# fabianschenk/REVO

Hardware: AMD Instinct MI355X
Metric: tracked frames/sec at 640x480, 4-level pyramid; ATE vs reference (higher is better)
Workload: dtype f32

## Files before the change

revo_amd/csrc/revo_host.hip:

```cpp
#include "revo_host_impl.h"

static thread_local std::string g_err;
extern "C" const char* revo_last_error(void) { return g_err.c_str(); }
extern "C" const char* revo_version(void) { return "0.1.0 gfx950"; }
extern "C" void revo_set_error_(const char* msg) { g_err = msg ? msg : ""; }

extern "C" void revo_pyr_settings_default(revo_pyr_settings* s) {
  memset(s, 0, sizeof(*s));
  s->width = 640; s->height = 480;
  s->fx = 517.306408f; s->fy = 516.469215f; s->cx = 318.643040f; s->cy = 255.313989f;
  s->pyr_min_lvl = 2; s->pyr_max_lvl = 0;
  s->canny_threshold1 = 150; s->canny_threshold2 = 100;
  s->depth_min = 0.1f; s->depth_max = 5.2f;
  s->use_edge_hist = 1; s->n_percentage = 0.3f;
  s->hist_patch[0] = 20; s->hist_patch[1] = 10; s->hist_patch[2] = 5;
}
extern "C" void revo_opt_settings_default(revo_opt_settings* s) {
  memset(s, 0, sizeof(*s));
  s->lambda_success_fac = 0.5f; s->lambda_fail_fac = 2.0f;
  const float ed[6] = {30, 20, 10, 5, 5, 5};
  for (int i = 0; i < REVO_L; ++i) {
    s->lambda_initial[i] = 0.f; s->step_size_min[i] = 1e-16f; s->convergence_eps[i] = 0.999f;
    s->max_its_per_lvl[i] = 100; s->edge_distance_lvl[i] = ed[i];
  }
  s->huber_edge = 0.3f;
  s->use_edge_filter = 1;
}
extern "C" void revo_tracker_settings_default(revo_tracker_settings* s) {
  s->check_tracking_results = 1; s->check_init_values = 1; s->n_frames_hist_voting = 3;
  s->histogram_level = 2;
}

static int build_geom(const revo_pyr_settings& s, PyrGeom* g, std::string* why) {
  memset(g, 0, sizeof(*g));
  g->fstride = 1;
  const int L = s.pyr_min_lvl - s.pyr_max_lvl + 1;
  if (s.pyr_max_lvl != 0) { *why = "pyr_max_lvl must be 0 (the reference indexes per-level vectors by level)"; return -1; }
  if (L < 1 || L > REVO_L) { *why = "1..6 pyramid levels supported"; return -1; }
  if (s.width <= 0 || s.height <= 0 || s.width > REVO_MAX_WIDTH || s.height > 2048 ||
      ((s.width + 31) / 32) * ((s.height + 31) / 32) > 2048) {
    *why = "image size must be within 2048 x 2048 and 2048 tiles of 32 x 32 pixels (1920 x 1080 fits, 2048 x 1536 does not)"; return -1;
  }
  if (s.width % (4 << (L - 1)) || s.height % (1 << (L - 1))) {
    *why = "width must be a multiple of 4*2^(levels-1) and height of 2^(levels-1)"; return -1;
  }
  g->n_levels = L;
  { const char* e = getenv("REVO_HYST_BANDED"); g->hyst_force = (e && *e) ? (*e != '0' ? 1 : 0) : -1; }
  g->hyst_heavy_runs = env_int("REVO_HYST_HEAVY_RUNS", 0, 0, 1 << 30);
  g->depth_min = s.depth_min; g->depth_max = s.depth_max;
  double lo = s.canny_threshold1, hi = s.canny_threshold2;
  if (lo > hi) std::swap(lo, hi);
  lo = std::min(32767.0, lo); hi = std::min(32767.0, hi);
  if (lo > 0) lo *= lo;
  if (hi > 0) hi *= hi;
  g->canny_low = (int)std::floor(lo); g->canny_high = (int)std::floor(hi);
  g->use_edge_hist = s.use_edge_hist; g->n_percentage = s.n_percentage;
  int tile = 0, pix = 0, row = 0, col = 0, cc = 0, tiles32 = 0, bands = 0;
  bool bands_fit = true;
  for (int l = 0; l < L; ++l) {
    LevelGeom& v = g->lv[l];
    const float scale = 1.0f / (float)std::pow(2, l);
    if (l == 0) { v.fx = s.fx; v.fy = s.fy; v.cx = s.cx; v.cy = s.cy; v.w = s.width; v.h = s.height; }
    else {
      v.fx = s.fx * scale; v.fy = s.fy * scale; v.cx = s.cx * scale; v.cy = s.cy * scale;
      v.w = (int)((float)s.width * scale); v.h = (int)((float)s.height * scale);
    }
    v.npix = v.w * v.h;
    if (v.npix % 16) { *why = "every level must have a multiple of 16 pixels"; return -1; }
    v.patch = s.hist_patch[l] > 0 ? s.hist_patch[l] : 0;
    if (v.patch > 0) {
      v.hist_w = v.w / v.patch; v.hist_h = v.h / v.patch;
      if (v.hist_w < 1 || v.hist_h < 1 || v.hist_w > 128) { *why = "hist_patch out of range for this level size"; return -1; }
    }
    g->fill_thr[l] = (double)(v.patch * v.patch) * 0.05;
    v.chunk_rows = 32; v.nchunk = (v.h + 31) / 32;
    v.wpr = (v.w + 31) / 32;
    v.nms_block_base = tile; tile += (8 * v.wpr * ((v.h + NMS_ROWS - 1) / NMS_ROWS) + 255) / 256;
    v.pix_base = pix; pix += v.npix;
    v.edt_rows = std::max(1, EDT_ROW_PX / v.w);
    v.edt_block_base = row; row += (v.h + v.edt_rows - 1) / v.edt_rows;
    v.strip_base = col; col += (v.w + 63) / 64;
    v.cc_base = cc; cc += v.w * v.nchunk;
    tiles32 += v.wpr * v.nchunk;
    {
      int unit = v.patch > 0 ? v.patch : 4;
      while (unit % 4) unit *= 2;
      int rows = (env_int("REVO_HYST_BAND_WORDS", 2400, 64, 1 << 20) / v.wpr) / unit * unit;
      if (rows < unit) rows = unit;
      if (rows >= v.h) rows = v.h;
      if ((v.h + rows - 1) / rows > 32) rows = ((v.h + 31) / 32 + unit - 1) / unit * unit;
      v.band_rows = rows;
      v.nbands = (v.h + rows - 1) / rows;
      v.band_base = bands; bands += v.nbands;
      if (v.nbands > 1) g->any_banded = 1;
      const size_t nwb = (size_t)rows * v.wpr;
      if (nwb + (nwb + 2) / 2 + (size_t)(rows + 2) * v.wpr + 2 + 256 > 16384) bands_fit = false;
    }
  }
  g->total_tiles = tiles32;
  g->total_bands = bands_fit ? bands : 0;
  for (int l = 1; l < L; ++l)
    g->lv[l].has_orig = (s.use_edge_hist && g->lv[l].patch > 0 && g->lv[l - 1].patch > 0) ? 1 : 0;
  g->total_nms_blocks = tile; g->total_pix = pix; g->total_edt_blocks = row; g->total_strips = col; g->total_cc = cc;
  return 0;
}

static void build_track_params(const revo_ctx* c, TrackParams* t) {
  memset(t, 0, sizeof(*t));
  t->pyr_min_lvl = c->ps.pyr_min_lvl; t->pyr_max_lvl = c->ps.pyr_max_lvl;
  t->lvl_begin = c->ps.pyr_min_lvl; t->lvl_end = c->ps.pyr_max_lvl;
  t->check_init = c->ts.check_init_values;
  t->lambda_success_fac = c->os.lambda_success_fac; t->lambda_fail_fac = c->os.lambda_fail_fac;
  for (int i = 0; i < REVO_L; ++i) {
    t->lambda_initial[i] = c->os.lambda_initial[i]; t->step_size_min[i] = c->os.step_size_min[i];
    t->convergence_eps[i] = c->os.convergence_eps[i]; t->max_its[i] = c->os.max_its_per_lvl[i];
    t->edge_distance[i] = c->os.edge_distance_lvl[i];
  }
  t->huber_edge = c->os.huber_edge; t->use_edge_filter = c->os.use_edge_filter;
  {
    const char* e = getenv("REVO_TRACK_KSPEC");
    const size_t n = e ? strlen(e) : 0;
    for (int i = 0; i < REVO_L; ++i) {
      int k = i < 2 ? 2 : TRACK_KMAX;
      if (n == 1) k = e[0] - '0'; else if (n > 1) k = e[std::min<size_t>(i, n - 1)] - '0';
      t->kspec[i] = std::max(1, std::min(TRACK_KMAX, k));
    }
  }
  t->redundant_n = env_int("REVO_TRACK_REDUNDANT_BATCH", 400, 0, 1 << 30);
  for (int l = 0; l < c->geom.n_levels; ++l) {
    const LevelGeom& v = c->geom.lv[l];
    t->cam[l].fx = v.fx; t->cam[l].fy = v.fy; t->cam[l].cx = v.cx; t->cam[l].cy = v.cy; t->cam[l].w = v.w; t->cam[l].h = v.h;
  }
}

static int env_track_depth() {
  const char* e = getenv("REVO_TRACK_SERIAL");
  if (e && *e && *e != '0') return 1;
  return env_int("REVO_TRACK_DEPTH", 2, 1, 4);
}
int pick_cluster(const revo_ctx* c, int n_pairs) {
  const int resident = c->num_cus * c->blocks_per_cu;
  const int depth = c->knobs.track_depth;
  const int share = n_pairs == 1 || depth == 1 ? (int)(0.75 * resident) : resident / depth;
  int cl = share / std::max(1, n_pairs);
  if (n_pairs == 1) cl = std::min(cl, 16);
  if (cl > TRACK_MAX_CLUSTER) cl = TRACK_MAX_CLUSTER;
  {
    const int want = n_pairs == 1 ? c->knobs.cluster_one : env_int("REVO_TRACK_CLUSTER", 0, 0, TRACK_MAX_CLUSTER);
    const int hard = std::min(TRACK_MAX_CLUSTER, resident / std::max(1, n_pairs));
    if (want >= 1) cl = std::min(want, std::max(1, hard));
  }
  if (cl < 1) cl = 1;
  return cl;
}

#define TRACK_MAX_DEPTH 4
struct TrackChain {
  std::mutex mu;
  hipEvent_t ev[TRACK_MAX_DEPTH] = {};
  hipStream_t st[TRACK_MAX_DEPTH] = {};
  bool has[TRACK_MAX_DEPTH] = {};
  unsigned long long n = 0;
// ... 332 lines not shown
```

revo_amd/csrc/revo_pyramid.hip:

```cpp
#include "revo_dev.h"
#include "revo_nms_px.h"
#include <type_traits>

namespace {

#ifdef REVO_BUILD_PRIO
#define BUILD_PRIO() __builtin_amdgcn_s_setprio(REVO_BUILD_PRIO)
#else
#define BUILD_PRIO()
#endif

__device__ __forceinline__ int level_of(const PyrGeom& g, int v, int LevelGeom::*base) {
  int l = 0;
#pragma unroll
  for (int k = 1; k < REVO_L; ++k)
    if (k < g.n_levels && v >= g.lv[k].*base) l = k;
  return l;
}
__device__ __forceinline__ int clampi(int v, int lo, int hi) { return v < lo ? lo : (v > hi ? hi : v); }
__device__ __forceinline__ int reflect101(int i, int n) {
  if (i < 0) i = -i;
  if (i >= n) i = 2 * n - 2 - i;
  return i;
}

__device__ __forceinline__ uint32_t gray4(uint32_t a, uint32_t b, uint32_t c) {
  const int B0 = a & 255, G0 = (a >> 8) & 255, R0 = (a >> 16) & 255, B1 = a >> 24;
  const int G1 = b & 255, R1 = (b >> 8) & 255, B2 = (b >> 16) & 255, G2 = b >> 24;
  const int R2 = c & 255, B3 = (c >> 8) & 255, G3 = (c >> 16) & 255, R3 = c >> 24;
  const uint32_t y0 = (uint32_t)(B0 * 1868 + G0 * 9617 + R0 * 4899 + 8192) >> 14;
  const uint32_t y1 = (uint32_t)(B1 * 1868 + G1 * 9617 + R1 * 4899 + 8192) >> 14;
  const uint32_t y2 = (uint32_t)(B2 * 1868 + G2 * 9617 + R2 * 4899 + 8192) >> 14;
  const uint32_t y3 = (uint32_t)(B3 * 1868 + G3 * 9617 + R3 * 4899 + 8192) >> 14;
  return y0 | (y1 << 8) | (y2 << 16) | (y3 << 24);
}
__global__ void __launch_bounds__(256) k_gray_depth(const uint8_t* __restrict__ bgr, const float* __restrict__ depth_f32,
                                                    const uint16_t* __restrict__ depth_u16, float alpha,
                                                    uint8_t* __restrict__ gray, float* __restrict__ depth_out, int npix, int frame0) {
  BUILD_PRIO();
  const int f = frame0 + blockIdx.z;
  const int g16 = blockIdx.x * 256 + threadIdx.x;
  if (g16 * 16 >= npix) return;
  const uint4* src = reinterpret_cast<const uint4*>(bgr + (size_t)f * npix * 3) + (size_t)g16 * 3;
  const uint4 p = src[0], q = src[1], r = src[2];
  reinterpret_cast<uint4*>(gray + (size_t)f * npix)[g16] =
      make_uint4(gray4(p.x, p.y, p.z), gray4(p.w, q.x, q.y), gray4(q.z, q.w, r.x), gray4(r.y, r.z, r.w));
  if (depth_out == depth_f32) return;
  float4* dst = reinterpret_cast<float4*>(depth_out + (size_t)f * npix) + (size_t)g16 * 4;
  if (depth_u16) {
    const uint4* raw = reinterpret_cast<const uint4*>(depth_u16 + (size_t)f * npix) + (size_t)g16 * 2;
    const uint4 u = raw[0], v = raw[1];
    const uint32_t wds[8] = {u.x, u.y, u.z, u.w, v.x, v.y, v.z, v.w};
#pragma unroll
    for (int k = 0; k < 4; ++k) {
      float4 d;
      d.x = (float)(wds[2 * k] & 0xffff) * alpha + 0.0f;
      d.y = (float)(wds[2 * k] >> 16) * alpha + 0.0f;
      d.z = (float)(wds[2 * k + 1] & 0xffff) * alpha + 0.0f;
      d.w = (float)(wds[2 * k + 1] >> 16) * alpha + 0.0f;
      dst[k] = d;
    }
  } else {
    const float4* in = reinterpret_cast<const float4*>(depth_f32 + (size_t)f * npix) + (size_t)g16 * 4;
    const float4 d0 = in[0], d1 = in[1], d2 = in[2], d3 = in[3];
    dst[0] = d0; dst[1] = d1; dst[2] = d2; dst[3] = d3;
  }
}

struct EdgeStage {
  const uint2* cs;
  const unsigned short* epre;
  const int* base;
  float* out;
  int wpr, tiles_total;
};
template <bool GRAY, bool DEPTH, bool STAGE = false>
__global__ void __launch_bounds__(256) k_pyrdown(const uint8_t* __restrict__ src, int sw, int sh, uint8_t* __restrict__ dst,
                                                 int dw, int dh, const float* __restrict__ dsrc, float* __restrict__ ddst, int frame0,
                                                 int fstride, uint8_t* __restrict__ vsrc, float dmin, float dmax, EdgeStage es) {
  BUILD_PRIO();
  static_assert(!STAGE || DEPTH, "staging rides on the depth half");
  const int f = frame0 + fstride * blockIdx.z;
  src += (size_t)f * sw * sh;
  dst += (size_t)f * dw * dh;
// ... 1525 lines not shown
  for (int o = 1; o < 64; o <<= 1) {
    const int v = __shfl_up(incl, o);
    if (lane >= o) incl += v;
  }
  if (lane == 63) s_part[wave] = incl;
  __syncthreads();
  int run = incl - sum, total = 0;
#pragma unroll
  for (int k = 0; k < 16; ++k) {
    const int wv = s_part[k];
    run += k < wave ? wv : 0;
    total += wv;
  }
  for (int i = b; i < e; ++i) { const int c = a[i]; a[i] = run; run += c; }
  return total;
}


__global__ void __launch_bounds__(256) k_pyrdown_bgr(const uint8_t* __restrict__ src, int w, int h,
                                                     uint8_t* __restrict__ dst) {
  const int dw = w >> 1, dh = h >> 1;
  const int i = blockIdx.x * 256 + threadIdx.x;
  if (i >= dw * dh) return;
  const int x = i % dw, y = i / dw;
  const int kk[5] = {1, 4, 6, 4, 1};
  int acc[3] = {0, 0, 0};
#pragma unroll
  for (int j = 0; j < 5; ++j) {
    const uint8_t* row = src + (size_t)reflect101(2 * y + j - 2, h) * w * 3;
    int rs[3] = {0, 0, 0};
#pragma unroll
    for (int t = 0; t < 5; ++t) {
      const uint8_t* px = row + (size_t)reflect101(2 * x + t - 2, w) * 3;
      rs[0] += kk[t] * px[0]; rs[1] += kk[t] * px[1]; rs[2] += kk[t] * px[2];
    }
    acc[0] += kk[j] * rs[0]; acc[1] += kk[j] * rs[1]; acc[2] += kk[j] * rs[2];
  }
  uint8_t* o = dst + (size_t)i * 3;
  o[0] = (uint8_t)((acc[0] + 128) >> 8); o[1] = (uint8_t)((acc[1] + 128) >> 8); o[2] = (uint8_t)((acc[2] + 128) >> 8);
}

template <bool WRITE>
__global__ void __launch_bounds__(256) k_pcl_walk(LevelGeom lv, float dmin, float dmax, const float* __restrict__ depth,
                                                  const uint8_t* __restrict__ edges, const uint8_t* __restrict__ bgr,
                                                  int dense, int* __restrict__ chunk, unsigned* __restrict__ cmask,
                                                  const int* __restrict__ total, int cap, float4* __restrict__ out) {
  const int i = blockIdx.x * 256 + threadIdx.x;
  if (i >= lv.w * lv.nchunk) return;
  const int x = i % lv.w, c = i / lv.w;
  const int yb = c * lv.chunk_rows, ye = min(lv.h, yb + lv.chunk_rows);
  const size_t slot = (size_t)x * lv.nchunk + c;
  if (!WRITE) {
    unsigned vm = 0;
    for (int y = yb; y < ye; ++y) {
      const size_t p = (size_t)y * lv.w + x;
      if ((dense || edges[p]) && depth_ok(depth[p], dmin, dmax)) vm |= 1u << (y - yb);
    }
    cmask[slot] = vm;
    chunk[slot] = __popc(vm);
  } else {
    if (*total > cap) return;
    int o = chunk[slot];
    for (unsigned m = cmask[slot]; m; m &= m - 1) {
      const int y = yb + __ffs(m) - 1;
      const size_t p = (size_t)y * lv.w + x;
      const float Z = depth[p];
      const float X = __fdiv_rn(Z * ((float)x - lv.cx), lv.fx);
      const float Y = __fdiv_rn(Z * ((float)y - lv.cy), lv.fy);
      const uint8_t* px = bgr + p * 3;
      out[2 * o] = make_float4(X, Y, Z, 1.0f);
      out[2 * o + 1] = make_float4(__fdiv_rn((float)px[2], 255.0f), __fdiv_rn((float)px[1], 255.0f),
                                   __fdiv_rn((float)px[0], 255.0f), 1.0f);
      ++o;
    }
  }
}

__global__ void __launch_bounds__(1024) k_pcl_scan(int* chunk, int n, int* total) {
  __shared__ int s_part[1024];
  const int t = block_exclusive_scan(chunk, n, s_part);
  if (threadIdx.x == 0) *total = t;
}

#define EDT_INF (1 << 29)
#define EDT_THREADS 1024
#define EDT_COL_GROUPS(h) ((h) > 1024 ? 64 : ((h) > 512 ? 32 : 16))
__global__ void __launch_bounds__(EDT_THREADS) k_edt_cols(PyrGeom g, FramePlanes pl, int f0, int fstride, int nframes) {
  __shared__ int s_first[EDT_THREADS];
  __shared__ int s_last[EDT_THREADS];
  const int f = f0 + (blockIdx.x % nframes) * fstride;
  int l = 0, sidx = blockIdx.x / nframes, ngroups = 16, ncols = 64;
  for (int k = 0; k < g.n_levels; ++k) {
    ngroups = EDT_COL_GROUPS(g.lv[k].h);
    ncols = EDT_THREADS / ngroups;
    const int ns = (g.lv[k].w + ncols - 1) / ncols;
    if (sidx < ns) { l = k; break; }
    sidx -= ns;
  }
  const LevelGeom& lv = g.lv[l];
  const int col = threadIdx.x % ncols, grp = threadIdx.x / ncols;
  const int x = sidx * ncols + col;
  const int rpg = (lv.h + ngroups - 1) / ngroups;
  const int yb = min(lv.h, grp * rpg), ye = min(lv.h, yb + rpg);
  const bool in = x < lv.w;
  const uint8_t* edges = pl.edges[l] + (size_t)f * lv.npix;
  unsigned em = 0;
  if ((lv.w & 31) == 0 && (ncols & 31) == 0) {
    const uint2* csw = pl.cs[l] + (size_t)f * lv.h * lv.wpr;
    const int r = threadIdx.x & 31;
    const int wc = (sidx * ncols + (col & ~31)) >> 5;
    uint32_t v = 0;
    if (yb + r < ye && wc < lv.wpr) v = csw[(size_t)(yb + r) * lv.wpr + wc].y;
    em = tile_transpose32(v, r);
    if (!in) em = 0;
  } else if (in) {
#pragma unroll 8
    for (int y = yb; y < ye; ++y) em |= (edges[(size_t)y * lv.w + x] ? 1u : 0u) << (y - yb);
  }
  s_first[grp * ncols + col] = em ? yb + __ffs(em) - 1 : EDT_INF;
  s_last[grp * ncols + col] = em ? yb + 31 - __clz(em) : -EDT_INF;
  __syncthreads();
  if (!in) return;
  int above = -EDT_INF, below = EDT_INF;
  for (int k = 0; k < grp; ++k) above = max(above, s_last[k * ncols + col]);
  for (int k = ngroups - 1; k > grp; --k) below = min(below, s_first[k * ncols + col]);
  uint16_t* gd = reinterpret_cast<uint16_t*>(pl.scratch[l]) + (size_t)f * lv.npix;
  const int FAR = 1 << 20;
  int du = (above <= -EDT_INF) ? FAR : (yb - above);
  const int dbelow = (below >= EDT_INF) ? FAR : (below - yb);
  for (int y = yb; y < ye; ++y) {
    const int k = y - yb;
    const unsigned hi = em >> k;
    du = (hi & 1u) ? 0 : du;
    const int dn = hi ? __ffs(hi) - 1 : dbelow - k;
    const int m = min(du, dn);
    gd[(size_t)y * lv.w + x] = (uint16_t)(m >= 0xffff ? 0xffff : m);
    du += 1;
  }
}

__device__ __forceinline__ float sqrt_rn_int(float x) {
  const float s = __builtin_amdgcn_sqrtf(x);
  const unsigned si = __float_as_uint(s);
  const float sd = __uint_as_float(si - 1u), su = __uint_as_float(si + 1u);
  const float rd = __builtin_fmaf(-sd, s, x), ru = __builtin_fmaf(-su, s, x);
  float r = (rd <= 0.0f) ? sd : s;
  r = (ru > 0.0f) ? su : r;
  return r;
}
__global__ void __launch_bounds__(256) k_edt_rows(PyrGeom g, FramePlanes pl, int f0, int fstride) {
  extern __shared__ int s_g2[];
  const int f = f0 + blockIdx.z * fstride;
  const int l = level_of(g, blockIdx.x, &LevelGeom::edt_block_base);
  const LevelGeom lv = g.lv[l];
  const int w = lv.w;
  const int y0 = (blockIdx.x - lv.edt_block_base) * lv.edt_rows;
  const int nr = min(lv.edt_rows, lv.h - y0);
  const int pad = w + 4, pitch = w + 2 * pad;
  const uint16_t* gd = reinterpret_cast<const uint16_t*>(pl.scratch[l]) + (size_t)f * lv.npix + (size_t)y0 * w;
  const int4 inf4 = make_int4(EDT_INF, EDT_INF, EDT_INF, EDT_INF);
  const int padq = pad >> 2, wq = w >> 2;
  for (int r = 0; r < nr; ++r) {
    int4* row4 = reinterpret_cast<int4*>(s_g2 + r * pitch);
    for (int i = threadIdx.x; i < padq; i += 256) { row4[i] = inf4; row4[padq + wq + i] = inf4; }
    const uint2* src = reinterpret_cast<const uint2*>(gd + r * w);
    for (int i = threadIdx.x; i < wq; i += 256) {
      const uint2 q = src[i];
      const int d0 = (int)(q.x & 0xffffu), d1 = (int)(q.x >> 16), d2 = (int)(q.y & 0xffffu), d3 = (int)(q.y >> 16);
      row4[padq + i] = make_int4(d0 == 0xffff ? EDT_INF : __mul24(d0, d0), d1 == 0xffff ? EDT_INF : __mul24(d1, d1),
                                 d2 == 0xffff ? EDT_INF : __mul24(d2, d2), d3 == 0xffff ? EDT_INF : __mul24(d3, d3));
    }
  }
  __syncthreads();
  float* dt = pl.dt[l] + (size_t)f * lv.npix + (size_t)y0 * w;
  const int dq = 256 / w, dr = 256 - dq * w;
  int r = threadIdx.x / w, x = threadIdx.x - r * w;
  for (int p = threadIdx.x; p < nr * w; p += 256) {
    const int* c = s_g2 + r * pitch + pad + x;
    int best = c[0];
    for (int d = 1; d < w && d * d < best; d += 4) {
      int m = best;
#pragma unroll
      for (int j = 0; j < 4; ++j) {
        const int dj = d + j;
        m = min(m, dj * dj + min(c[-dj], c[dj]));
      }
      best = m;
    }
    dt[p] = best >= EDT_INF ? sqrtf(1e15f) : sqrt_rn_int((float)best);
    x += dr; r += dq;
    if (x >= w) { x -= w; ++r; }
  }
}

__global__ void __launch_bounds__(256) k_grad_table(PyrGeom g, FramePlanes pl, int f0, int fstride) {
  const int f = f0 + blockIdx.z * fstride;
  const int l = blockIdx.y;
  const LevelGeom& lv = g.lv[l];
  const int i = blockIdx.x * 256 + threadIdx.x;
  if (i >= lv.npix) return;
  const float* dt = pl.dt[l] + (size_t)f * lv.npix;
  float4 o = make_float4(0.f, 0.f, 0.f, 0.f);
  if (i >= lv.w && i < lv.w * (lv.h - 1)) {
    o.x = 0.5f * (dt[i - 1] - dt[i + 1]);
    o.y = 0.5f * (dt[i - lv.w] - dt[i + lv.w]);
    o.z = dt[i];
  }
  pl.table[l][(size_t)f * lv.npix + i] = o;
}

__global__ void __launch_bounds__(256) k_vote_mark(VoteArgs a, float fx, float fy, float cx, float cy, int W, int H,
                                                   int* marks) {
  const int c = blockIdx.y;
  const int n = *a.n[c];
  const float* R = a.RT[c];
  const float* T = R + 9;
  const float4* pts = a.pts[c];
  for (int i = blockIdx.x * 256 + threadIdx.x; i < n; i += gridDim.x * 256) {
    const float4 p = pts[i];
    float q[3];
#pragma unroll
    for (int r = 0; r < 3; ++r) q[r] = ((R[r] * p.x + R[3 + r] * p.y) + R[6 + r] * p.z) + T[r];
    const float u = __fdiv_rn(fx * q[0], q[2]) + cx;
    const float v = __fdiv_rn(fy * q[1], q[2]) + cy;
    if (u >= 0 && u < (float)W && v >= 0 && v < (float)H)
      atomicOr(&marks[(int)floorf(v) * W + (int)floorf(u)], 1 << c);
  }
}

__global__ void __launch_bounds__(256) k_vote_hist(int* marks, const uint8_t* edges, const float* depth, int npix,
                                                   float dmin, float dmax, int* hist8, unsigned* done, int* host_out,
                                                   unsigned seq_val) {
  __shared__ int s_h[8];
  __shared__ bool s_last;
  if (threadIdx.x < 8) s_h[threadIdx.x] = 0;
  __syncthreads();
  for (int i = blockIdx.x * 256 + threadIdx.x; i < npix; i += gridDim.x * 256) {
    const int m = marks[i];
    if (m) marks[i] = 0;
    const float Z = depth[i];
    if (depth_ok(Z, dmin, dmax)) {
      const int val = __popc(m);
      atomicAdd(&s_h[val], 1);
      if (edges[i] > 0) atomicAdd(&s_h[4 + val], 1);
    }
  }
  __syncthreads();
  if (threadIdx.x < 8 && s_h[threadIdx.x]) atomicAdd(&hist8[threadIdx.x], s_h[threadIdx.x]);
  __threadfence();
  __syncthreads();
  if (threadIdx.x == 0) s_last = (atomicAdd(done, 1u) == gridDim.x - 1);
  __syncthreads();
  if (s_last) {
    if (threadIdx.x < 8) host_out[threadIdx.x] = atomicExch(&hist8[threadIdx.x], 0);
    if (threadIdx.x == 0) *done = 0u;
    __threadfence_system();
    __syncthreads();
    if (threadIdx.x == 0) *(volatile int*)&host_out[8] = (int)seq_val;
  }
}

__global__ void __launch_bounds__(256) k_copy_cloud(float4* __restrict__ dst, const float4* __restrict__ src,
                                                    int* __restrict__ dst_n, const int* __restrict__ src_n) {
  const int n = *src_n;
  for (int i = blockIdx.x * 256 + threadIdx.x; i < n; i += gridDim.x * 256) dst[i] = src[i];
  if (blockIdx.x == 0 && threadIdx.x == 0) *dst_n = n;
}

__global__ void __launch_bounds__(256) k_vote_mark_multi(const VoteDesc* __restrict__ descs, float fx, float fy, float cx,
                                                         float cy, int W, int H) {
  const VoteDesc& d = descs[blockIdx.z];
  const int c = blockIdx.y;
  if (c >= d.n_clouds) return;
  const int n = *d.n[c];
// ... 146 lines not shown
  }
  const bool mixed = !banded && fits_single && g.hyst_heavy_runs > 0 && g.total_bands > 0 && g.lv[0].nbands > 1;
  if (mixed) {
    static bool attr3 = false;
    if (!attr3) {
      (void)hipFuncSetAttribute(reinterpret_cast<const void*>(k_hyst_mixed), hipFuncAttributeMaxDynamicSharedMemorySize, REVO_HYST_LDS_MAX);
      (void)hipFuncSetAttribute(reinterpret_cast<const void*>(k_hyst_out), hipFuncAttributeMaxDynamicSharedMemorySize, HB_LDS_WORDS * 4);
      (void)hipFuncSetAttribute(reinterpret_cast<const void*>(k_hyst_seam), hipFuncAttributeMaxDynamicSharedMemorySize, 64 * 1024);
      (void)hipGetLastError();
      attr3 = true;
    }
    const LevelGeom& l0 = g.lv[0];
    const size_t seam_lds = std::max<size_t>(4, (size_t)l0.nbands * (size_t)(HB_LDS_WORDS / 2 / 32 + 64) * 4);
    const size_t out_lds = std::max<size_t>(4, (size_t)l0.band_rows * l0.wpr * 4);
    hipLaunchKernelGGL(k_hyst_mixed, dim3((l0.nbands + g.n_levels) * B), dim3(HYST_THREADS), REVO_HYST_LDS_MAX, s, g, p, B);
    hipLaunchKernelGGL(k_hyst_seam, dim3(B), dim3(HS_THREADS), seam_lds, s, g, p, 1);
    hipLaunchKernelGGL(k_hyst_out, dim3(l0.nbands * B), dim3(HO_THREADS), out_lds, s, g, p, 1);
    hipLaunchKernelGGL(k_hyst<true>, dim3(std::min(32, g.n_levels * B)), dim3(HYST_THREADS), REVO_HYST_LDS_MAX, s, g, p, 1, B);
    return;
  }
  const int n_wg = only_flagged ? std::min(32, g.n_levels * B) : g.n_levels * B;
  if (ec_bytes + 4096 <= REVO_HYST_LDS_MAX)
    hipLaunchKernelGGL(k_hyst<true>, dim3(n_wg), dim3(HYST_THREADS), REVO_HYST_LDS_MAX, s, g, p, only_flagged, B);
  else if (e_bytes <= REVO_HYST_LDS_MAX)
    hipLaunchKernelGGL(k_hyst<false>, dim3(n_wg), dim3(HYST_THREADS), e_bytes, s, g, p, only_flagged, B);
  else
    hipLaunchKernelGGL((k_hyst<false, true>), dim3(n_wg), dim3(HYST_THREADS), 16, s, g, p, only_flagged, B);
}

void launch_fill(const PyrGeom& g, const FramePlanes& p, int B, hipStream_t s) {
  bool any = false;
  for (int l = 1; l < g.n_levels; ++l) any = any || g.lv[l].has_orig;
  if (!any) return;
  if (g.lv[0].npix <= 640 * 480) {
    hipLaunchKernelGGL(k_fill, dim3(1, 1, B), dim3(1024), 0, s, g, p, 0);
    return;
  }
  for (int l = 1; l < g.n_levels; ++l) {
    if (!g.lv[l].has_orig) continue;
    const int n = (g.lv[l - 1].w / 2) * (g.lv[l - 1].h / 2);
    hipLaunchKernelGGL(k_fill, dim3(std::min(64, (n + 1023) / 1024), 1, B), dim3(1024), 0, s, g, p, l);
  }
}

void launch_tile_points(const PyrGeom& g, const FramePlanes& p, int B, hipStream_t s, int which) {
  if (which & 1) hipLaunchKernelGGL(k_tile_count, dim3(g.n_levels * B), dim3(1024), 0, s, g, p);
  const int groups = (g.total_tiles + PT_TILES - 1) / PT_TILES;
  if ((which & 2) && g.pts_staged) hipLaunchKernelGGL(k_pts_tiles<true>, dim3(groups * B), dim3(32 * PT_TILES), 0, s, g, p);
  else if (which & 2) hipLaunchKernelGGL(k_pts_tiles<false>, dim3(groups * B), dim3(32 * PT_TILES), 0, s, g, p);
}

void launch_compact(const PyrGeom& g, const FramePlanes& p, int B, hipStream_t s) {
  dim3 grid(g.total_strips * B);
  hipLaunchKernelGGL(k_compact_walk<false>, grid, dim3(CW_COLS * CW_LANES_COUNT), 0, s, g, p);
  hipLaunchKernelGGL(k_compact_walk<true>, grid, dim3(CW_COLS * CW_LANES), 0, s, g, p);
}

void launch_pyrdown_bgr(const uint8_t* src, int w, int h, uint8_t* dst, hipStream_t s) {
  hipLaunchKernelGGL(k_pyrdown_bgr, dim3(((w / 2) * (h / 2) + 255) / 256), dim3(256), 0, s, src, w, h, dst);
}

void launch_colored_pcl(const PyrGeom& g, const FramePlanes& p, int frame, int lvl, int dense, const uint8_t* bgr_lvl,
                        int* chunk, unsigned* cmask, int* total, int cap, float* out8, hipStream_t s) {
  const LevelGeom& lv = g.lv[lvl];
  const float* depth = p.depth[lvl] + (size_t)frame * lv.npix;
  const uint8_t* edges = p.edges[lvl] + (size_t)frame * lv.npix;
  const int n = lv.w * lv.nchunk;
  dim3 grid((n + 255) / 256);
  hipLaunchKernelGGL(k_pcl_walk<false>, grid, dim3(256), 0, s, lv, g.depth_min, g.depth_max, depth, edges, bgr_lvl, dense,
                     chunk, cmask, total, cap, (float4*)out8);
  hipLaunchKernelGGL(k_pcl_scan, dim3(1), dim3(1024), 0, s, chunk, n, total);
  hipLaunchKernelGGL(k_pcl_walk<true>, grid, dim3(256), 0, s, lv, g.depth_min, g.depth_max, depth, edges, bgr_lvl, dense,
                     chunk, cmask, total, cap, (float4*)out8);
}

void launch_keyframe(const PyrGeom& g, const FramePlanes& p, int f0, int fstride, int count, hipStream_t s, int which) {
  int strips = 0;
  for (int l = 0; l < g.n_levels; ++l) {
    const int ncols = EDT_THREADS / EDT_COL_GROUPS(g.lv[l].h);
    strips += (g.lv[l].w + ncols - 1) / ncols;
  }
  if (which & 1) hipLaunchKernelGGL(k_edt_cols, dim3(strips * count), dim3(EDT_THREADS), 0, s, g, p, f0, fstride, count);
  size_t rows_lds = 0;
  for (int l = 0; l < g.n_levels; ++l) rows_lds = std::max(rows_lds, (size_t)g.lv[l].edt_rows * (3 * g.lv[l].w + 8) * sizeof(int));
  if (which & 2) hipLaunchKernelGGL(k_edt_rows, dim3(g.total_edt_blocks, 1, count), dim3(256), rows_lds, s, g, p, f0, fstride);
}

void launch_grad_table(const PyrGeom& g, const FramePlanes& p, int f0, int fstride, int count, hipStream_t s) {
  hipLaunchKernelGGL(k_grad_table, dim3((g.lv[0].npix + 255) / 256, g.n_levels, count), dim3(256), 0, s, g, p, f0, fstride);
}

void launch_vote(const PyrGeom& g, const FramePlanes& curr, int curr_frame, int lvl, int n_clouds, const VoteArgs& va,
                 int* d_marks, int* d_hist8, unsigned* d_done, int* h_out8, unsigned seq_val, int use_orig_edges, hipStream_t s) {
  const LevelGeom& lv = g.lv[lvl];
  if (n_clouds > 0)
    hipLaunchKernelGGL(k_vote_mark, dim3(32, n_clouds), dim3(256), 0, s, va, lv.fx, lv.fy, lv.cx, lv.cy, lv.w, lv.h, d_marks);
  const uint8_t* edges = (use_orig_edges ? curr.edges_orig[lvl] : curr.edges[lvl]) + (size_t)curr_frame * lv.npix;
  hipLaunchKernelGGL(k_vote_hist, dim3(16), dim3(256), 0, s, d_marks, edges,
                     curr.depth[lvl] + (size_t)curr_frame * lv.npix, lv.npix, g.depth_min, g.depth_max, d_hist8, d_done, h_out8,
                     seq_val);
}

void launch_copy_cloud(float4* dst, const float4* src, int* dst_n, const int* src_n, hipStream_t s) {
  hipLaunchKernelGGL(k_copy_cloud, dim3(16), dim3(256), 0, s, dst, src, dst_n, src_n);
}

void launch_vote_multi(const PyrGeom& g, int lvl, int n, const VoteDesc* d_descs, unsigned seq_val, hipStream_t s) {
  const LevelGeom& lv = g.lv[lvl];
  hipLaunchKernelGGL(k_vote_mark_multi, dim3(32, 3, n), dim3(256), 0, s, d_descs, lv.fx, lv.fy, lv.cx, lv.cy, lv.w, lv.h);
  hipLaunchKernelGGL(k_vote_hist_multi, dim3(16, n), dim3(256), 0, s, d_descs, lv.npix, g.depth_min, g.depth_max, seq_val);
}

void launch_copy_cloud_multi(int n, const CloudCopyDesc* d_descs, hipStream_t s) {
  hipLaunchKernelGGL(k_copy_cloud_multi, dim3(16, n), dim3(256), 0, s, d_descs);
}

void launch_copy_segments(int n, const CopySeg* d_segs, hipStream_t s) {
  hipLaunchKernelGGL(k_copy_segments, dim3(64, n), dim3(256), 0, s, d_segs);
}
```

Before: 118,300.

## Pack two rows into 16-bit lanes for EDT row pass with 32-bit fallback

The row pass of the distance transform now stores squared column distances as saturated 16-bit values, packing two image rows per 32-bit LDS word. It searches both rows at once with packed min and saturating add, capped at a reach of 256 pixels, and ends the search early when the whole wavefront agrees via ballot. If any pixel stays saturated, the block reruns the old exact 32-bit search, so results stay exact. This aims to halve LDS traffic and ALU work per pixel and to shrink the LDS footprint. The cost is extra code, an even row count per block, and a possible second pass.

Measured after the change: 118,900 (median of 4 runs). Within noise of the previous version (+0.5%).

```diff
diff --git a/profiles/edt_isa_counts.py b/profiles/edt_isa_counts.py
--- /dev/null
+++ b/profiles/edt_isa_counts.py
@@ -0,0 +1,88 @@
+#!/usr/bin/env python3
+import argparse
+import os
+import re
+import shutil
+import subprocess
+import sys
+import tempfile
+
+sys.path.insert(0, os.path.dirname(os.path.abspath(__file__)))
+from nms_isa_counts import NOT_ALU, ROOT, assembly, count
+
+KERNEL = "k_edt_rows"
+TRIP = 4
+LDS_WORDS = {"ds_read_b32": 1, "ds_read2_b32": 2, "ds_read_b64": 2, "ds_read2_b64": 4, "ds_read_b96": 3, "ds_read_b128": 4,
+             "ds_read_u16": 1, "ds_read_u8": 1}
+
+
+def loops(asm):
+    m = re.search(r"^(_Z\w*%s\w*):[^\n]*\n(.*?)^\s*\.section\s+\.rodata" % KERNEL, asm, re.S | re.M)
+    if not m:
+        raise SystemExit("kernel %s not found in the assembly" % KERNEL)
+    inner, order, cur = {}, [], None
+    for ln in m.group(2).splitlines():
+        lab = re.match(r"^\.LBB\d+_(\d+):", ln)
+        if lab or ln.startswith("; %bb."):
+            cur = None
+            if lab:
+                cur_label = lab.group(1)
+        hdr = re.search(r"in Loop: Header=BB\d+_(\d+) Depth=(\d+)", ln)
+        if hdr:
+            cur = hdr.group(1)
+        if "Inner Loop Header" in ln:
+            cur = cur_label
+            order.append(cur)
+        op = ln.split(";")[0].strip()
+        if not op or op.startswith(".") or op.endswith(":") or cur is None:
+            continue
+        inner.setdefault(cur, []).append(op.split()[0])
+    return [inner[k] for k in order if any(o.startswith("ds_read") for o in inner.get(k, []))]
+
+
+def loop_counts(ops):
+    packed = any(o.startswith("v_pk_min_u16") for o in ops)
+    c = {"kind": "packed" if packed else "32-bit", "px": 2 if packed else 1,
+         "VALU": sum(o.startswith("v_") for o in ops),
+         "SALU": sum(o.startswith("s_") and not o.startswith(NOT_ALU) for o in ops),
+         "LDS instructions": sum(o.startswith("ds_") for o in ops),
+         "LDS words": sum(LDS_WORDS.get(o, 0) for o in ops),
+         "branches": sum(o.startswith(("s_branch", "s_cbranch")) for o in ops)}
+    return c
+
+
+def report(name, asm):
+    c = count(asm, KERNEL)
+    lds = re.search(r"\.amdhsa_group_segment_fixed_size (\d+)", asm[asm.index(".amdhsa_kernel _ZN12_GLOBAL__N_110%s" % KERNEL):])
+    print("%s: k_edt_rows, gfx950" % name)
+    print("  whole kernel: %d instructions, %d VALU, %d SALU, %d memory, %d branches; VGPRs in use %d, scratch %d bytes, static LDS %s "
+          "bytes (the rows are dynamic LDS: launch_keyframe)" % (c["instructions"], c["VALU"], c["SALU"], c["memory"], c["branches"],
+                                                                c["VGPRs"], c["scratch bytes"], lds.group(1) if lds else "?"))
+    for ops in loops(asm):
+        k = loop_counts(ops)
+        n = TRIP * k["px"]
+        print("  %-6s trip loop: %2d VALU, %2d SALU, %d LDS instructions = %d words, %d branches per trip of %d distances x %d pixel(s)"
+              "  ->  %.2f VALU, %.2f SALU, %.2f LDS words per pixel and distance" % (
+                  k["kind"], k["VALU"], k["SALU"], k["LDS instructions"], k["LDS words"], k["branches"], TRIP, k["px"],
+                  k["VALU"] / n, k["SALU"] / n, k["LDS words"] / n))
+
+
+def main():
+    ap = argparse.ArgumentParser(description=__doc__, formatter_class=argparse.RawDescriptionHelpFormatter)
+    ap.add_argument("--rev", action="append", default=[], help="also count this commit's sources (repeatable)")
+    ap.add_argument("--keep", help="write the working tree's revo_pyramid.s into this directory")
+    a = ap.parse_args()
+    for rev in a.rev:
+        tmp = tempfile.mkdtemp(prefix="edt_isa_src_")
+        tar = subprocess.run(["git", "-C", ROOT, "archive", rev, "revo_amd/csrc", "include"], check=True, stdout=subprocess.PIPE).stdout
+        subprocess.run(["tar", "-x", "-C", tmp], input=tar, check=True)
+        report(rev, assembly(os.path.join(tmp, "revo_amd", "csrc")))
+        shutil.rmtree(tmp)
+    if a.keep:
+        os.makedirs(a.keep, exist_ok=True)
+    report("working tree", assembly(os.path.join(ROOT, "revo_amd", "csrc"), a.keep))
+    return 0
+
+
+if __name__ == "__main__":
+    sys.exit(main())
diff --git a/revo_amd/csrc/revo_edt_px.h b/revo_amd/csrc/revo_edt_px.h
--- /dev/null
+++ b/revo_amd/csrc/revo_edt_px.h
@@ -0,0 +1,96 @@
+#pragma once
+#include <math.h>
+#include <stdint.h>
+
+#if defined(__HIPCC__) || defined(__CUDACC__)
+#define EDT_HD __host__ __device__ __forceinline__
+#else
+#define EDT_HD inline
+#endif
+
+#define EDT_INF (1 << 29)
+#define EDT_PK_SAT 0xffffu
+#define EDT_PK_REACH 256
+#define EDT_TRIP 4
+
+EDT_HD uint32_t edt_sq16(uint32_t g) { return g > 255u ? EDT_PK_SAT : g * g; }
+EDT_HD int edt_sq32(uint32_t g) { return g == 0xffffu ? EDT_INF : (int)(g * g); }
+EDT_HD uint32_t edt_pack(uint32_t lo, uint32_t hi) { return lo | hi << 16; }
+#define EDT_PK_NO_PARTNER 0u
+
+#if defined(__HIP_DEVICE_COMPILE__)
+typedef unsigned short edt_us2 __attribute__((ext_vector_type(2)));
+EDT_HD uint32_t edt_pk_min(uint32_t a, uint32_t b) {
+  return __builtin_bit_cast(uint32_t, __builtin_elementwise_min(__builtin_bit_cast(edt_us2, a), __builtin_bit_cast(edt_us2, b)));
+}
+EDT_HD uint32_t edt_pk_add_sat(uint32_t a, uint32_t b) {
+  return __builtin_bit_cast(uint32_t, __builtin_elementwise_add_sat(__builtin_bit_cast(edt_us2, a), __builtin_bit_cast(edt_us2, b)));
+}
+EDT_HD uint32_t edt_pk_sub_sat(uint32_t a, uint32_t b) {
+  return __builtin_bit_cast(uint32_t, __builtin_elementwise_sub_sat(__builtin_bit_cast(edt_us2, a), __builtin_bit_cast(edt_us2, b)));
+}
+#else
+EDT_HD uint32_t edt_h_min(uint32_t a, uint32_t b) { return a < b ? a : b; }
+EDT_HD uint32_t edt_pk_min(uint32_t a, uint32_t b) {
+  return edt_pack(edt_h_min(a & 0xffffu, b & 0xffffu), edt_h_min(a >> 16, b >> 16));
+}
+EDT_HD uint32_t edt_pk_add_sat(uint32_t a, uint32_t b) {
+  return edt_pack(edt_h_min((a & 0xffffu) + (b & 0xffffu), EDT_PK_SAT), edt_h_min((a >> 16) + (b >> 16), EDT_PK_SAT));
+}
+EDT_HD uint32_t edt_pk_sub_sat(uint32_t a, uint32_t b) {
+  const uint32_t al = a & 0xffffu, bl = b & 0xffffu, ah = a >> 16, bh = b >> 16;
+  return edt_pack(al > bl ? al - bl : 0u, ah > bh ? ah - bh : 0u);
+}
+#endif
+
+EDT_HD uint32_t edt_pk_dd(int d) {
+  const uint32_t dd = (uint32_t)(d * d);
+  return (dd < EDT_PK_SAT ? dd : EDT_PK_SAT) * 0x10001u;
+}
+EDT_HD bool edt_pk_more(uint32_t best, int d) { return edt_pk_sub_sat(best, edt_pk_dd(d)) != 0u; }
+EDT_HD uint32_t edt_pk_trip(const uint32_t* c, int d, uint32_t best) {
+#if defined(__HIP_DEVICE_COMPILE__)
+#pragma unroll
+#endif
+  for (int j = 0; j < EDT_TRIP; ++j) {
+    const int dj = d + j;
+    best = edt_pk_min(best, edt_pk_add_sat(edt_pk_min(c[-dj], c[dj]), edt_pk_dd(dj)));
+  }
+  return best;
+}
+EDT_HD int edt_pk_dmax(int w) { return w < EDT_PK_REACH ? w : EDT_PK_REACH; }
+EDT_HD int edt_pk_pad(int w) { return edt_pk_dmax(w) + EDT_TRIP; }
+EDT_HD bool edt_pk_undecided(uint32_t best) { return (best & 0xffffu) == EDT_PK_SAT || (best >> 16) == EDT_PK_SAT; }
+
+EDT_HD int edt_search32(const int* c, int w) {
+  int best = c[0];
+  for (int d = 1; d < w && d * d < best; d += EDT_TRIP) {
+    int m = best;
+#if defined(__HIP_DEVICE_COMPILE__)
+#pragma unroll
+#endif
+    for (int j = 0; j < EDT_TRIP; ++j) {
+      const int dj = d + j;
+      const int l = c[-dj], r = c[dj];
+      const int t = dj * dj + (l < r ? l : r);
+      m = t < m ? t : m;
+    }
+    best = m;
+  }
+  return best;
+}
+
+EDT_HD float sqrt_rn_int(float x) {
+#if defined(__HIP_DEVICE_COMPILE__)
+  const float s = __builtin_amdgcn_sqrtf(x);
+#else
+  const float s = sqrtf(x);
+#endif
+  const uint32_t si = __builtin_bit_cast(uint32_t, s);
+  const float sd = __builtin_bit_cast(float, si - 1u), su = __builtin_bit_cast(float, si + 1u);
+  const float rd = __builtin_fmaf(-sd, s, x), ru = __builtin_fmaf(-su, s, x);
+  float r = (rd <= 0.0f) ? sd : s;
+  r = (ru > 0.0f) ? su : r;
+  return r;
+}
+EDT_HD float edt_value(int d2) { return d2 >= EDT_INF ? sqrtf(1e15f) : sqrt_rn_int((float)d2); }
diff --git a/revo_amd/csrc/revo_host.hip b/revo_amd/csrc/revo_host.hip
--- a/revo_amd/csrc/revo_host.hip
+++ b/revo_amd/csrc/revo_host.hip
@@ -77,7 +77,7 @@
     v.wpr = (v.w + 31) / 32;
     v.nms_block_base = tile; tile += (8 * v.wpr * ((v.h + NMS_ROWS - 1) / NMS_ROWS) + 255) / 256;
     v.pix_base = pix; pix += v.npix;
-    v.edt_rows = std::max(1, EDT_ROW_PX / v.w);
+    v.edt_rows = std::max(2, (EDT_ROW_PX / v.w) & ~1);
     v.edt_block_base = row; row += (v.h + v.edt_rows - 1) / v.edt_rows;
     v.strip_base = col; col += (v.w + 63) / 64;
     v.cc_base = cc; cc += v.w * v.nchunk;
diff --git a/revo_amd/csrc/revo_pyramid.hip b/revo_amd/csrc/revo_pyramid.hip
--- a/revo_amd/csrc/revo_pyramid.hip
+++ b/revo_amd/csrc/revo_pyramid.hip
@@ -1,5 +1,6 @@
 #include "revo_dev.h"
 #include "revo_nms_px.h"
+#include "revo_edt_px.h"
 #include <type_traits>
 
 namespace {
@@ -1691,7 +1692,6 @@
   if (threadIdx.x == 0) *total = t;
 }
 
-#define EDT_INF (1 << 29)
 #define EDT_THREADS 1024
 #define EDT_COL_GROUPS(h) ((h) > 1024 ? 64 : ((h) > 512 ? 32 : 16))
 __global__ void __launch_bounds__(EDT_THREADS) k_edt_cols(PyrGeom g, FramePlanes pl, int f0, int fstride, int nframes) {
@@ -1748,57 +1748,83 @@
   }
 }
 
-__device__ __forceinline__ float sqrt_rn_int(float x) {
-  const float s = __builtin_amdgcn_sqrtf(x);
-  const unsigned si = __float_as_uint(s);
-  const float sd = __uint_as_float(si - 1u), su = __uint_as_float(si + 1u);
-  const float rd = __builtin_fmaf(-sd, s, x), ru = __builtin_fmaf(-su, s, x);
-  float r = (rd <= 0.0f) ? sd : s;
-  r = (ru > 0.0f) ? su : r;
-  return r;
-}
+__device__ __forceinline__ int edt_fb_rows(int w, int rows) { return min(rows, max(1, EDT_ROW_PX / w)); }
+__host__ __device__ inline int edt_pk_words(int w, int rows) { return edt_pk_pad(w) + ((rows + 1) >> 1) * (w + edt_pk_pad(w)); }
+__host__ __device__ inline int edt_fb_words(int w, int rows) { return (w + EDT_TRIP) + rows * (2 * w + EDT_TRIP); }
 __global__ void __launch_bounds__(256) k_edt_rows(PyrGeom g, FramePlanes pl, int f0, int fstride) {
-  extern __shared__ int s_g2[];
+  extern __shared__ uint32_t s_edt[];
   const int f = f0 + blockIdx.z * fstride;
   const int l = level_of(g, blockIdx.x, &LevelGeom::edt_block_base);
   const LevelGeom lv = g.lv[l];
-  const int w = lv.w;
+  const int w = lv.w, wq = w >> 2;
   const int y0 = (blockIdx.x - lv.edt_block_base) * lv.edt_rows;
   const int nr = min(lv.edt_rows, lv.h - y0);
-  const int pad = w + 4, pitch = w + 2 * pad;
   const uint16_t* gd = reinterpret_cast<const uint16_t*>(pl.scratch[l]) + (size_t)f * lv.npix + (size_t)y0 * w;
-  const int4 inf4 = make_int4(EDT_INF, EDT_INF, EDT_INF, EDT_INF);
-  const int padq = pad >> 2, wq = w >> 2;
-  for (int r = 0; r < nr; ++r) {
-    int4* row4 = reinterpret_cast<int4*>(s_g2 + r * pitch);
-    for (int i = threadIdx.x; i < padq; i += 256) { row4[i] = inf4; row4[padq + wq + i] = inf4; }
-    const uint2* src = reinterpret_cast<const uint2*>(gd + r * w);
-    for (int i = threadIdx.x; i < wq; i += 256) {
-      const uint2 q = src[i];
-      const int d0 = (int)(q.x & 0xffffu), d1 = (int)(q.x >> 16), d2 = (int)(q.y & 0xffffu), d3 = (int)(q.y >> 16);
-      row4[padq + i] = make_int4(d0 == 0xffff ? EDT_INF : __mul24(d0, d0), d1 == 0xffff ? EDT_INF : __mul24(d1, d1),
-                                 d2 == 0xffff ? EDT_INF : __mul24(d2, d2), d3 == 0xffff ? EDT_INF : __mul24(d3, d3));
-    }
-  }
-  __syncthreads();
   float* dt = pl.dt[l] + (size_t)f * lv.npix + (size_t)y0 * w;
   const int dq = 256 / w, dr = 256 - dq * w;
-  int r = threadIdx.x / w, x = threadIdx.x - r * w;
-  for (int p = threadIdx.x; p < nr * w; p += 256) {
-    const int* c = s_g2 + r * pitch + pad + x;
-    int best = c[0];
-    for (int d = 1; d < w && d * d < best; d += 4) {
-      int m = best;
-#pragma unroll
-      for (int j = 0; j < 4; ++j) {
-        const int dj = d + j;
-        m = min(m, dj * dj + min(c[-dj], c[dj]));
-      }
-      best = m;
-    }
-    dt[p] = best >= EDT_INF ? sqrtf(1e15f) : sqrt_rn_int((float)best);
-    x += dr; r += dq;
-    if (x >= w) { x -= w; ++r; }
+  const int r_t = threadIdx.x / w, x_t = threadIdx.x - r_t * w;
+  bool undecided = false;
+  {
+    const int np = (nr + 1) >> 1;
+    const int pad = edt_pk_pad(w), pitch = w + pad, padq = pad >> 2;
+    const uint4 sat4 = make_uint4(~0u, ~0u, ~0u, ~0u);
+    for (int i = threadIdx.x; i < padq; i += 256) reinterpret_cast<uint4*>(s_edt)[i] = sat4;
+    for (int k = 0; k < np; ++k) {
+      uint4* row4 = reinterpret_cast<uint4*>(s_edt + pad + k * pitch);
+      for (int i = threadIdx.x; i < padq; i += 256) row4[wq + i] = sat4;
+      const uint2* src = reinterpret_cast<const uint2*>(gd + 2 * k * w);
+      const bool lower = 2 * k + 1 < nr;
+      for (int i = threadIdx.x; i < wq; i += 256) {
+        const uint2 a = src[i];
+        uint4 v = make_uint4(edt_sq16(a.x & 0xffffu), edt_sq16(a.x >> 16), edt_sq16(a.y & 0xffffu), edt_sq16(a.y >> 16));
+        if (lower) {
+          const uint2 b = src[wq + i];
+          v.x = edt_pack(v.x, edt_sq16(b.x & 0xffffu)); v.y = edt_pack(v.y, edt_sq16(b.x >> 16));
+          v.z = edt_pack(v.z, edt_sq16(b.y & 0xffffu)); v.w = edt_pack(v.w, edt_sq16(b.y >> 16));
+        }
+        row4[i] = v;
+      }
+    }
+    __syncthreads();
+    const int dmax = edt_pk_dmax(w);
+    const int dci = dq * pitch + dr, dco = 2 * dq * w + dr;
+    int x = x_t, ci = pad + r_t * pitch + x_t, o = 2 * r_t * w + x_t;
+    for (int p = threadIdx.x; p < np * w; p += 256) {
+      const uint32_t* c = s_edt + ci;
+      uint32_t best = c[0];
+      for (int d = 1; d < dmax && __builtin_amdgcn_ballot_w64(edt_pk_more(best, d)) != 0; d += EDT_TRIP) best = edt_pk_trip(c, d, best);
+      undecided |= edt_pk_undecided(best);
+      dt[o] = sqrt_rn_int((float)(best & 0xffffu));
+      if (o + w < nr * w) dt[o + w] = sqrt_rn_int((float)(best >> 16));
+      x += dr; ci += dci; o += dco;
+      if (x >= w) { x -= w; ci += pad; o += w; }
+    }
+  }
+  if (!__syncthreads_or(undecided)) return;
+  int* s_g2 = reinterpret_cast<int*>(s_edt);
+  const int pad = w + EDT_TRIP, pitch = w + pad, padq = pad >> 2;
+  const int fr = edt_fb_rows(w, lv.edt_rows);
+  const int4 inf4 = make_int4(EDT_INF, EDT_INF, EDT_INF, EDT_INF);
+  for (int r0 = 0; r0 < nr; r0 += fr) {
+    const int n = min(fr, nr - r0);
+    if (r0) __syncthreads();
+    for (int i = threadIdx.x; i < padq; i += 256) reinterpret_cast<int4*>(s_g2)[i] = inf4;
+    for (int r = 0; r < n; ++r) {
+      int4* row4 = reinterpret_cast<int4*>(s_g2 + pad + r * pitch);
+      for (int i = threadIdx.x; i < padq; i += 256) row4[wq + i] = inf4;
+      const uint2* src = reinterpret_cast<const uint2*>(gd + (r0 + r) * w);
+      for (int i = threadIdx.x; i < wq; i += 256) {
+        const uint2 q = src[i];
+        row4[i] = make_int4(edt_sq32(q.x & 0xffffu), edt_sq32(q.x >> 16), edt_sq32(q.y & 0xffffu), edt_sq32(q.y >> 16));
+      }
+    }
+    __syncthreads();
+    int x = x_t, ci = pad + r_t * pitch + x_t;
+    for (int p = threadIdx.x; p < n * w; p += 256) {
+      dt[r0 * w + p] = edt_value(edt_search32(s_g2 + ci, w));
+      x += dr; ci += dq * pitch + dr;
+      if (x >= w) { x -= w; ci += pad; }
+    }
   }
 }
 
@@ -2111,7 +2137,11 @@
   }
   if (which & 1) hipLaunchKernelGGL(k_edt_cols, dim3(strips * count), dim3(EDT_THREADS), 0, s, g, p, f0, fstride, count);
   size_t rows_lds = 0;
-  for (int l = 0; l < g.n_levels; ++l) rows_lds = std::max(rows_lds, (size_t)g.lv[l].edt_rows * (3 * g.lv[l].w + 8) * sizeof(int));
+  for (int l = 0; l < g.n_levels; ++l) {
+    const int w = g.lv[l].w, rows = g.lv[l].edt_rows;
+    const int words = std::max(edt_pk_words(w, rows), edt_fb_words(w, std::min(rows, std::max(1, EDT_ROW_PX / w))));
+    rows_lds = std::max(rows_lds, (size_t)words * sizeof(int));
+  }
   if (which & 2) hipLaunchKernelGGL(k_edt_rows, dim3(g.total_edt_blocks, 1, count), dim3(256), rows_lds, s, g, p, f0, fstride);
 }
 
```
